# parrot-tts/Parrot-TTS

Hardware: AMD Instinct MI355X
Metric: audio samples/sec (16 kHz; see config.note) + RTF, 256-unit batch-64 per GPU (higher is better)
Workload: dtype f32 (f16x3 split products)

## Files before the change

parrot_tts_amd/csrc/conv_split.h:

```cpp
#pragma once
#include <cstdlib>
#include <type_traits>

#include "conv_mfma.h"

namespace parrot {

typedef short s16x8 __attribute__((ext_vector_type(8)));
typedef __bf16 bf16x8 __attribute__((ext_vector_type(8)));
typedef _Float16 f16x8 __attribute__((ext_vector_type(8)));

typedef __bf16 bf16x2 __attribute__((ext_vector_type(2)));
typedef _Float16 f16x2 __attribute__((ext_vector_type(2)));
typedef float f32x2 __attribute__((ext_vector_type(2)));
__device__ __forceinline__ unsigned pk_bf16(float x0, float x1) {
    const f32x2 v = {x0, x1};
    return __builtin_bit_cast(unsigned, __builtin_convertvector(v, bf16x2));
}
__device__ __forceinline__ unsigned pk_f16(float x0, float x1) {
    const f32x2 v = {x0, x1};
    return __builtin_bit_cast(unsigned, __builtin_convertvector(v, f16x2));
}
__device__ __forceinline__ float max_nc(float a, float b) {
    float r;
// ... 27 lines not shown
        const f32x2 v = {x0, x1};
        q[0] = __builtin_bit_cast(unsigned, __builtin_convertvector(v, f16x2));
        float r0, r1;
        asm("v_fma_mix_f32 %0, %1, -1.0, %2 op_sel_hi:[1,0,0]" : "=v"(r0) : "v"(q[0]), "v"(x0));
        asm("v_fma_mix_f32 %0, %1, -1.0, %2 op_sel:[1,0,0] op_sel_hi:[1,0,0]" : "=v"(r1) : "v"(q[0]), "v"(x1));
        q[1] = pk_f16(r0, r1);
    }
};
struct SchBf16 {
    static constexpr int ID = 3, NP = 1, NT = 1;
    static constexpr bool F16 = false;
    static constexpr float XS = 1.f;
    static constexpr int pa(int) { return 0; }
    static constexpr int pb(int) { return 0; }
    static constexpr int last_a(int) { return 0; }
    static __device__ __forceinline__ void split(float x0, float x1, unsigned (&q)[1]) { q[0] = pk_bf16(x0, x1); }
};
struct SchF16 {
    static constexpr int ID = 4, NP = 1, NT = 1;
    static constexpr bool F16 = true;
    static constexpr float XS = 8.f;
    static constexpr int pa(int) { return 0; }
    static constexpr int pb(int) { return 0; }
    static constexpr int last_a(int) { return 0; }
    static __device__ __forceinline__ void split(float x0, float x1, unsigned (&q)[1]) { q[0] = pk_f16(x0, x1); }
};

template <class SCH>
__device__ __forceinline__ f32x16 mfma32(const s16x8& a, const s16x8& b, const f32x16& c) {
    if constexpr (SCH::F16) return __builtin_amdgcn_mfma_f32_32x32x16_f16(__builtin_bit_cast(f16x8, a), __builtin_bit_cast(f16x8, b), c, 0, 0, 0);
    else return __builtin_amdgcn_mfma_f32_32x32x16_bf16(__builtin_bit_cast(bf16x8, a), __builtin_bit_cast(bf16x8, b), c, 0, 0, 0);
}
template <class SCH>
__device__ __forceinline__ f32x4 mfma16(const s16x8& a, const s16x8& b, const f32x4& c) {
    if constexpr (SCH::F16) return __builtin_amdgcn_mfma_f32_16x16x32_f16(__builtin_bit_cast(f16x8, a), __builtin_bit_cast(f16x8, b), c, 0, 0, 0);
    else return __builtin_amdgcn_mfma_f32_16x16x32_bf16(__builtin_bit_cast(bf16x8, a), __builtin_bit_cast(bf16x8, b), c, 0, 0, 0);
}
template <class SCH>
__device__ __forceinline__ float pre_scale(float v, float slope) {
    if constexpr (SCH::XS != 1.f) return max_nc(v * SCH::XS, v * (SCH::XS * slope));
    else return max_nc(v, v * slope);
}

template <int N, class F>
__device__ __forceinline__ void static_for(F&& f) {
    if constexpr (N > 0) {
        static_for<N - 1>(f);
        f(std::integral_constant<int, N - 1>{});
    }
}

template <class SCH, int WAVES_M, int WAVES_N, int WM, int WN, int MINW, int K, int SUBS = 1, bool LEAN = false>
__global__ __launch_bounds__(WAVES_M* WAVES_N * 64, MINW) void conv_split_kernel(const ConvParams p) {
    static_assert(SUBS == 1 || K == 1, "sub-slab staging: 1x1 convs only (no halo)");
    constexpr int NPC = SCH::NP, NTERM = SCH::NT;
    constexpr int NW = WAVES_M * WAVES_N, NT = NW * 64;
    constexpr int BM = WAVES_M * WM * 32;
    constexpr int BN = WAVES_N * WN * 32;
    constexpr int COLS = BN + ((SUBS > 1 && K == 1) ? 0 : CONV_HALO);
    constexpr int PIECE_BYTES = COLS * 32;
    constexpr int SUB_BYTES = NPC * PIECE_BYTES;
    constexpr int BUF_BYTES = SUBS * SUB_BYTES;
    constexpr int LIVE = SUBS * COLS * 2;
    constexpr int ITEMS = (LIVE + NT - 1) / NT;
    constexpr int KS = K * SUBS;
    constexpr int STEP_BYTES = NPC * 1024;

    extern __shared__ __attribute__((aligned(16))) char smem_raw[];

    const int tid = threadIdx.x;
    const int lane = tid & 63;
    const int wave = __builtin_amdgcn_readfirstlane(tid >> 6);
    const int wm = wave / WAVES_N;
    const int wn = wave % WAVES_N;
    const int half = lane >> 5;
    const int l31 = lane & 31;

    const int n_mb = (p.M + BM - 1) / BM;
    const int n_tiles = p.tiles_n * p.B, tpx = (n_tiles + 7) >> 3;
    const int xcd = blockIdx.x & 7, seq = blockIdx.x >> 3;
    const int mblock = seq % n_mb;
    const int tile_id = xcd * tpx + seq / n_mb;
    if (tile_id >= n_tiles || seq / n_mb >= tpx) return;
    const int b = tile_id / p.tiles_n;
    const int tn = tile_id - b * p.tiles_n;
    const int t0 = tn * BN;
    const int Tlim = p.row_len ? min(p.Tin, row_true_len(p.row_len[b], p.row_len_mul, p.row_len_add)) : p.Tin;
    const int W = BN + (p.k - 1) * p.dil;
    const int grp = (p.groups > 1) ? (mblock * BM) / p.Mg : 0;
    const float* __restrict__ xb = p.x + (size_t)b * p.x_bstride + (size_t)grp * p.Cin * p.Tin;

    static_assert(COLS % 64 == 0, "channel octet must be wave-uniform");
    const size_t xaddr = reinterpret_cast<size_t>(xb);
    const unsigned x_lo = __builtin_amdgcn_readfirstlane((unsigned)xaddr), x_hi = __builtin_amdgcn_readfirstlane((unsigned)(xaddr >> 32));
    const __amdgpu_buffer_rsrc_t xrsrc = __builtin_amdgcn_make_buffer_rsrc(
        reinterpret_cast<void*>(((size_t)x_hi << 32) | x_lo), 0, 0x7fffffff, 0x00020000);
    const int row_bytes = p.Tin * 4;
    const float slope = (p.pre == PRE_LRELU) ? p.pre_slope : 1.f;
    int voff[ITEMS], soct[ITEMS];
    static_for<ITEMS>([&](auto ic) {
        constexpr int i = decltype(ic)::value;
        const int item = tid + NT * i;
        const int so = item / COLS;
        const int col = item - so * COLS;
        const int tin = t0 - p.pad_left + col;
        voff[i] = (item < LIVE && col < W && tin >= 0 && tin < Tlim) ? tin * 4 : (int)0x80000000;
        soct[i] = __builtin_amdgcn_readfirstlane(min(so, 2 * SUBS - 1) * 8) * row_bytes;
// ... 23 lines not shown
                const int off = sub * SUB_BYTES + col * 32 + ((oct ^ ((col >> 3) & 1)) * 16);
#pragma unroll
                for (int pc = 0; pc < NPC; ++pc)
                    *reinterpret_cast<uint4*>(dst + pc * PIECE_BYTES + off) = uint4{q[0][pc], q[1][pc], q[2][pc], q[3][pc]};
            }
        });
    };

    f32x16 acc[WM][WN];
    const int m_wave = mblock * BM + wm * WM * 32;
    const int n_wave = t0 + wn * WN * 32;
    if constexpr (LEAN) conv_acc_init_lean<WM, WN>(p, acc, b, m_wave, n_wave, half, l31);
    else conv_acc_init<WM, WN>(p, acc, b, m_wave, n_wave, half, l31);

    const unsigned w_lo = __builtin_amdgcn_readfirstlane((unsigned)reinterpret_cast<size_t>(p.wfrag));
    const unsigned w_hi = __builtin_amdgcn_readfirstlane((unsigned)(reinterpret_cast<size_t>(p.wfrag) >> 32));
    const __amdgpu_buffer_rsrc_t wrsrc =
        __builtin_amdgcn_make_buffer_rsrc(reinterpret_cast<void*>(((size_t)w_hi << 32) | w_lo), 0, 0x7fffffff, 0x00020000);
    int abase[WM];
#pragma unroll
    for (int mt = 0; mt < WM; ++mt)
        abase[mt] = __builtin_amdgcn_readfirstlane((int)((mblock * (BM / 32) + wm * WM + mt) * p.n_it * STEP_BYTES));
    const unsigned lane16 = lane * 16;
    const int nsup = p.nchunks / SUBS;
    const int colbase = wn * WN * 32 + l31;
    auto load_b = [&](s16x8 (&bb)[WN][NPC], const char* __restrict__ xs, int tap) {
        const int col = colbase + tap * p.dil;
        const int off = col * 32 + ((half ^ ((col >> 3) & 1)) * 16);
#pragma unroll
        for (int nt = 0; nt < WN; ++nt)
#pragma unroll
            for (int pc = 0; pc < NPC; ++pc) bb[nt][pc] = *reinterpret_cast<const s16x8*>(xs + pc * PIECE_BYTES + nt * 1024 + off);
    };
    constexpr int TM = WM * WN, NMF = NTERM * TM;
    if constexpr (K > 0) {
        s16x8 A[2][WM][NPC], Bv[2][WN][NPC];
        auto load_a_piece = [&](s16x8 (&a)[WM][NPC], int pc, int soff) {
#pragma unroll
            for (int mt = 0; mt < WM; ++mt)
                a[mt][pc] = __builtin_bit_cast(s16x8, __builtin_amdgcn_raw_buffer_load_b128(wrsrc, lane16 + pc * 1024, abase[mt] + soff, 0));
        };
        auto next_chunk = [&](int q) { return (q + 1 == nsup) ? 0 : q + 1; };
        int cc = 0, cn = next_chunk(0);
#pragma unroll
        for (int pc = 0; pc < NPC; ++pc) {
            load_a_piece(A[0], pc, cc * KS * STEP_BYTES);
            load_a_piece(A[1], pc, (KS > 1 ? cc * KS + 1 : cn * KS) * STEP_BYTES);
        }
        load_slab(0);
        store_slab(0);
        __syncthreads();
        auto chunk = [&](auto par, int c) __attribute__((always_inline)) {
            constexpr int PAR = decltype(par)::value;
            const char* __restrict__ xs = smem_raw + (c & 1) * BUF_BYTES;
            const int cn2 = next_chunk(cn);
            load_slab(cn);
            load_b(Bv[PAR], xs, 0);
#pragma unroll
            for (int j = 0; j < KS; ++j) {
                const int cur = (PAR + j) & 1;
                const int tq = (j + 2 < KS) ? cc : (KS == 1 ? cn2 : cn);
                const int tj = (j + 2 < KS) ? j + 2 : (KS == 1 ? 0 : j + 2 - KS);
                const int soff = (tq * KS + tj) * STEP_BYTES;
                if (j + 1 < KS) load_b(Bv[cur ^ 1], xs + ((j + 1) / K) * SUB_BYTES, (j + 1) % K);
#pragma unroll
                for (int t = 0; t < NTERM; ++t) {
#pragma unroll
                    for (int mt = 0; mt < WM; ++mt)
#pragma unroll
                        for (int nt = 0; nt < WN; ++nt)
                            acc[mt][nt] = mfma32<SCH>(A[cur][mt][SCH::pa(t)], Bv[cur][nt][SCH::pb(t)], acc[mt][nt]);
#pragma unroll
                    for (int pc = 0; pc < NPC; ++pc)
                        if (t == SCH::last_a(pc)) load_a_piece(A[cur], pc, soff);
                }
            }
            constexpr int DS_START = (NPC >= 2) ? (SCH::last_a(NPC - 1) + 1) * TM - 1 + WM : 0;
            constexpr int SLAB_START = (NPC >= 2) ? (SCH::last_a(1) + 1) * TM - 1 + WM : 0;
            constexpr int SLAB_SLOTS = (NMF - SLAB_START) > 0 ? (NMF - SLAB_START) : 1, SLAB_PER = (ITEMS * 8 + SLAB_SLOTS - 1) / SLAB_SLOTS;
#pragma unroll
            for (int i = 0; i < NPC * WN; ++i) __builtin_amdgcn_sched_group_barrier(0x100, 1, 0);
#pragma unroll
            for (int j = 0; j < KS; ++j) {
                int ds_left = (j + 1 < KS) ? NPC * WN : 0, slab_left = (j == 0) ? ITEMS * 8 : 0;
#pragma unroll
                for (int m = 0; m < NMF; ++m) {
                    __builtin_amdgcn_sched_group_barrier(0x008, 1, 0);
#pragma unroll
                    for (int pc = NPC - 1; pc >= 1; --pc)
                        if (m >= (SCH::last_a(pc) + 1) * TM - 1 && m < (SCH::last_a(pc) + 1) * TM - 1 + WM) __builtin_amdgcn_sched_group_barrier(0x020, 1, 0);
                    if (m >= DS_START && ds_left > 0) {
                        __builtin_amdgcn_sched_group_barrier(0x100, 1, 0);
                        --ds_left;
                    }
                    if (m >= SLAB_START)
#pragma unroll
                        for (int q = 0; q < SLAB_PER; ++q)
                            if (slab_left > 0) {
                                __builtin_amdgcn_sched_group_barrier(0x020, 1, 0);
                                --slab_left;
                            }
                }
#pragma unroll
                for (int i = 0; i < WM; ++i) __builtin_amdgcn_sched_group_barrier(0x020, 1, 0);
            }
            __builtin_amdgcn_sched_barrier(0);
            store_slab((c + 1) & 1);
            __syncthreads();
            cc = cn;
            cn = cn2;
        };
        for (int c = 0; c < nsup; c += 2) {
            chunk(std::integral_constant<int, 0>{}, c);
            if (c + 1 < nsup) chunk(std::integral_constant<int, (KS & 1)>{}, c + 1);
        }
    } else {
        s16x8 a0[WM][NPC], b0[WN][NPC], a1[WM][NPC], b1[WN][NPC];
        auto load_a = [&](s16x8 (&a)[WM][NPC], int step) {
            const int soff = __builtin_amdgcn_readfirstlane(step) * STEP_BYTES;
#pragma unroll
            for (int mt = 0; mt < WM; ++mt)
#pragma unroll
                for (int pc = 0; pc < NPC; ++pc)
                    a[mt][pc] = __builtin_bit_cast(s16x8, __builtin_amdgcn_raw_buffer_load_b128(wrsrc, lane16 + pc * 1024, abase[mt] + soff, 0));
        };
        auto mfmas = [&](const s16x8 (&a)[WM][NPC], const s16x8 (&bb)[WN][NPC]) {
#pragma unroll
            for (int t = 0; t < NTERM; ++t)
#pragma unroll
                for (int mt = 0; mt < WM; ++mt)
#pragma unroll
                    for (int nt = 0; nt < WN; ++nt) acc[mt][nt] = mfma32<SCH>(a[mt][SCH::pa(t)], bb[nt][SCH::pb(t)], acc[mt][nt]);
        };
        load_a(a0, 0);
        load_slab(0);
        store_slab(0);
        __syncthreads();

        int cc = 0, cn = (1 == p.nchunks) ? 0 : 1;
        int c = 0, j = 0;
        const char* __restrict__ xs = smem_raw;
        auto step = [&](s16x8 (&xa)[WM][NPC], s16x8 (&xb)[WN][NPC], s16x8 (&ya)[WM][NPC], s16x8 (&yb)[WN][NPC]) {
            if (j == 0) {
                if (c + 1 < p.nchunks) load_slab(cn);
                load_b(xb, xs, 0);
            }
            const bool last_tap = (j + 1 == p.k);
            load_a(ya, last_tap ? cn * p.k : cc * p.k + j + 1);
            load_b(yb, xs, j + 1);
            mfmas(xa, xb);
            constexpr int MPER = (NMF / (NPC * (WM + WN))) > 0 ? (NMF / (NPC * (WM + WN))) : 1;
#pragma unroll
            for (int g = 0; g < WM * NPC; ++g) {
                __builtin_amdgcn_sched_group_barrier(0x008, MPER, 0);
                __builtin_amdgcn_sched_group_barrier(0x020, 1, 0);
            }
#pragma unroll
            for (int g = 0; g < WN * NPC; ++g) {
                __builtin_amdgcn_sched_group_barrier(0x008, MPER, 0);
                __builtin_amdgcn_sched_group_barrier(0x100, 1, 0);
            }
            __builtin_amdgcn_sched_barrier(0);
            if (last_tap) {
                if (c + 1 < p.nchunks) store_slab((c + 1) & 1);
                __syncthreads();
                ++c;
                xs = smem_raw + (c & 1) * BUF_BYTES;
                cc = cn;
                cn = (cc + 1 == p.nchunks) ? 0 : cc + 1;
                j = 0;
            } else {
                ++j;
            }
        };
        const int total = p.nchunks * p.k;
        for (int st = 0; st < total; st += 2) {
            step(a0, b0, a1, b1);
            if (st + 1 < total) step(a1, b1, a0, b0);
        }
    }
    if constexpr (LEAN) conv_epilogue_lean<WM, WN>(p, acc, b, m_wave, n_wave, half, l31);
    else conv_epilogue<WM, WN>(p, acc, b, m_wave, n_wave, half, l31);
}

template <class SCH, int WAVES_M, int WAVES_N, int WM, int WN, int MINW, int K, int SUBS = 1, bool LEAN = false>
inline hipError_t launch_conv_split_t(const ConvParams& p, dim3 grid, hipStream_t s) {
    constexpr int BN = WAVES_N * WN * 32;
    const size_t lds = (size_t)2 * SUBS * SCH::NP * (BN + ((SUBS > 1 && K == 1) ? 0 : CONV_HALO)) * 32;
    auto kern = conv_split_kernel<SCH, WAVES_M, WAVES_N, WM, WN, MINW, K, SUBS, LEAN>;
    static DynLdsOnce lds_once;
    {
        hipError_t e = ensure_dyn_lds(lds_once, reinterpret_cast<const void*>(kern), (size_t)lds);
        if (e != hipSuccess) return e;
    }
    hipLaunchKernelGGL(kern, grid, dim3(WAVES_M * WAVES_N * 64), lds, s, p);
    return hipGetLastError();
}

inline void split_tile(int variant, int& bm, int& bn) {
    if (variant == 2) { bm = 128; bn = 64; return; }
    if (variant == 3) { bm = 32; bn = 512; return; }
    bm = (variant & 1) ? 64 : 128;
    bn = (variant & 1) ? 256 : 128;
}
inline unsigned split_grid(const ConvParams& p, int bm) {
    const unsigned tiles = (unsigned)p.tiles_n * p.B, n_mb = (p.M + bm - 1) / bm;
    return (tiles + 7) / 8 * 8 * n_mb;
}
template <class SCH>
inline hipError_t launch_conv_split_s(int variant, const ConvParams& p, hipStream_t s) {
    int bm, bn;
    split_tile(variant, bm, bn);
    dim3 grid(split_grid(p, bm));
    if (variant == 3) return p.k == 3 ? launch_conv_split_t<SCH, 1, 4, 1, 4, 2, 3>(p, grid, s) : launch_conv_split_t<SCH, 1, 4, 1, 4, 2, 0>(p, grid, s);
    const bool lean = conv_lean_ok(p);
    if constexpr (SCH::ID == SchF16x3::ID) if (variant == 2) {
        if (p.k == 1 && p.nchunks % 4 == 0)
            return lean ? launch_conv_split_t<SCH, 4, 1, 1, 2, 3, 1, 4, true>(p, grid, s) : launch_conv_split_t<SCH, 4, 1, 1, 2, 3, 1, 4>(p, grid, s);
        switch (p.k) {
            case 1: return launch_conv_split_t<SCH, 4, 1, 1, 2, 3, 1>(p, grid, s);
            case 3: return launch_conv_split_t<SCH, 4, 1, 1, 2, 3, 3>(p, grid, s);
            case 9: return launch_conv_split_t<SCH, 4, 1, 1, 2, 3, 9>(p, grid, s);
            default: return launch_conv_split_t<SCH, 4, 1, 1, 2, 3, 0>(p, grid, s);
        }
    }
    if constexpr (SCH::ID != SchF16x3::ID) if (variant == 2) {
        if (p.k == 1 && p.nchunks % 4 == 0)
            return lean ? launch_conv_split_t<SCH, 2, 2, 2, 1, 3, 1, 4, true>(p, grid, s) : launch_conv_split_t<SCH, 2, 2, 2, 1, 3, 1, 4>(p, grid, s);
        switch (p.k) {
            case 1: return launch_conv_split_t<SCH, 2, 2, 2, 1, 3, 1>(p, grid, s);
            case 3: return launch_conv_split_t<SCH, 2, 2, 2, 1, 3, 3>(p, grid, s);
            case 9: return launch_conv_split_t<SCH, 2, 2, 2, 1, 3, 9>(p, grid, s);
            default: return launch_conv_split_t<SCH, 2, 2, 2, 1, 3, 0>(p, grid, s);
        }
    }
    if (variant & 1) switch (p.k) {
            case 1: return launch_conv_split_t<SCH, 1, 4, 2, 2, 2, 1>(p, grid, s);
            case 3: return launch_conv_split_t<SCH, 1, 4, 2, 2, 2, 3>(p, grid, s);
            case 7: return launch_conv_split_t<SCH, 1, 4, 2, 2, 2, 7>(p, grid, s);
            case 11: return launch_conv_split_t<SCH, 1, 4, 2, 2, 2, 11>(p, grid, s);
            default: return launch_conv_split_t<SCH, 1, 4, 2, 2, 2, 0>(p, grid, s);
        }
    switch (p.k) {
        case 3:
            return lean ? launch_conv_split_t<SCH, 2, 2, 2, 2, 2, 3, 1, true>(p, grid, s) : launch_conv_split_t<SCH, 2, 2, 2, 2, 2, 3>(p, grid, s);
        case 7: return launch_conv_split_t<SCH, 2, 2, 2, 2, 2, 7>(p, grid, s);
        case 9: return launch_conv_split_t<SCH, 2, 2, 2, 2, 2, 9>(p, grid, s);
        case 11: return launch_conv_split_t<SCH, 2, 2, 2, 2, 2, 11>(p, grid, s);
        default: return launch_conv_split_t<SCH, 2, 2, 2, 2, 2, 0>(p, grid, s);
    }
}
template <class SCH>
inline hipError_t launch_conv_split_generic(int variant, const ConvParams& p, hipStream_t s) {
    int bm, bn;
    split_tile(variant, bm, bn);
    dim3 grid(split_grid(p, bm));
    if (variant == 3) return launch_conv_split_t<SCH, 1, 4, 1, 4, 2, 0>(p, grid, s);
    if (variant == 2) {
        if (p.k == 1 && p.nchunks % 4 == 0) return launch_conv_split_t<SCH, 2, 2, 2, 1, 3, 1, 4>(p, grid, s);
        return launch_conv_split_t<SCH, 2, 2, 2, 1, 3, 0>(p, grid, s);
    }
    if (variant & 1) return launch_conv_split_t<SCH, 1, 4, 2, 2, 2, 0>(p, grid, s);
    return launch_conv_split_t<SCH, 2, 2, 2, 2, 2, 0>(p, grid, s);
}
hipError_t launch_conv_split_f16x3(int variant, const ConvParams& p, hipStream_t s);
hipError_t launch_conv_split_bf16x6(int variant, const ConvParams& p, hipStream_t s);
hipError_t launch_conv_split_bf16(int variant, const ConvParams& p, hipStream_t s);
hipError_t launch_conv_split_f16(int variant, const ConvParams& p, hipStream_t s);
inline hipError_t launch_conv_split(int scheme, int variant, const ConvParams& p, hipStream_t s) {
    switch (scheme) {
        case SchBf16x6::ID: return launch_conv_split_bf16x6(variant, p, s);
        case SchF16x3::ID: return launch_conv_split_f16x3(variant, p, s);
        case SchBf16::ID: return launch_conv_split_bf16(variant, p, s);
        case SchF16::ID: return launch_conv_split_f16(variant, p, s);
        default: return hipErrorInvalidValue;
    }
}

}
```

parrot_tts_amd/csrc/conv_valu.h:

```cpp
#pragma once
#include "conv_mfma.h"

namespace parrot {

struct ConvValuParams {
    const float* x;
    const float* w;
    const float* bias;
    float* y;
    int B, Cin, Tin, Tout;
    float slope;
    int act;
    const int32_t* row_len;
    int row_len_mul;
    int row_len_add;
    int* err;
};

__device__ __forceinline__ __amdgpu_buffer_rsrc_t valu_row_rsrc(const float* base) {
    const size_t a = reinterpret_cast<size_t>(base);
    const unsigned lo = __builtin_amdgcn_readfirstlane((unsigned)a), hi = __builtin_amdgcn_readfirstlane((unsigned)(a >> 32));
    return __builtin_amdgcn_make_buffer_rsrc(reinterpret_cast<void*>(((size_t)hi << 32) | lo), 0, 0x7fffffff, 0x00020000);
}

__global__ __launch_bounds__(256) void linear1_valu_kernel(const ConvValuParams p) {
    __shared__ float part[4][64];
    const int lane = threadIdx.x & 63, wave = threadIdx.x >> 6;
    const int b = blockIdx.y;
    const int t = blockIdx.x * 64 + lane;
    const int Tlim = p.row_len ? min(p.Tin, row_true_len(p.row_len[b], p.row_len_mul, p.row_len_add)) : p.Tin;
    const __amdgpu_buffer_rsrc_t xr = valu_row_rsrc(p.x + (size_t)b * p.Cin * p.Tin);
    const int voff = (t < Tlim) ? t * 4 : (int)0x80000000;
    const int per = (p.Cin + 3) / 4, c0 = wave * per, c1 = min(p.Cin, c0 + per);
    const int row_bytes = p.Tin * 4;
    float acc = 0.f;
    for (int c = c0; c < c1; ++c) {
        const float xv = __builtin_bit_cast(float, __builtin_amdgcn_raw_buffer_load_b32(xr, voff, c * row_bytes, 0));
        acc = fmaf(p.w[c], fmaxf(xv, xv * p.slope), acc);
    }
    part[wave][lane] = acc;
    __syncthreads();
    if (wave == 0 && t < p.Tout) {
        const float v = (((p.bias ? p.bias[0] : 0.f) + part[0][lane]) + part[1][lane]) + (part[2][lane] + part[3][lane]);
        if (p.act == ACT_TANH && p.err && !(fabsf(v) < INFINITY)) atomicExch(p.err, 5);
        p.y[(size_t)b * p.Tout + t] = (p.act == ACT_TANH) ? tanhf(v) : v;
    }
}

template <int K>
__global__ __launch_bounds__(256) void conv1_valu_kernel(const ConvValuParams p) {
    constexpr int NV = 4 + K - 1;
    const int b = blockIdx.y;
    const int t0 = (blockIdx.x * 256 + threadIdx.x) * 4;
    const int Tlim = p.row_len ? min(p.Tin, row_true_len(p.row_len[b], p.row_len_mul, p.row_len_add)) : p.Tin;
    const __amdgpu_buffer_rsrc_t xr = valu_row_rsrc(p.x + (size_t)b * p.Cin * p.Tin);
    int voff[NV];
#pragma unroll
    for (int i = 0; i < NV; ++i) {
        const int t = t0 - (K - 1) / 2 + i;
        voff[i] = (t >= 0 && t < Tlim) ? t * 4 : (int)0x80000000;
    }
    const float b0 = p.bias ? p.bias[0] : 0.f;
    float acc[4] = {b0, b0, b0, b0};
    const int row_bytes = p.Tin * 4;
    for (int c = 0; c < p.Cin; ++c) {
        float v[NV];
#pragma unroll
        for (int i = 0; i < NV; ++i) {
            const float xv = __builtin_bit_cast(float, __builtin_amdgcn_raw_buffer_load_b32(xr, voff[i], c * row_bytes, 0));
            v[i] = fmaxf(xv, xv * p.slope);
        }
#pragma unroll
        for (int j = 0; j < K; ++j) {
            const float wj = p.w[c * K + j];
#pragma unroll
            for (int o = 0; o < 4; ++o) acc[o] = fmaf(wj, v[o + j], acc[o]);
        }
    }
// ... 57 lines not shown
template <int COUT, int K, int U, int PAD>
__global__ __launch_bounds__(256) void convt_valu_kernel(const ConvValuParams p) {
    constexpr int DLO = -((K - 1 - PAD + U - 1) / U), DHI = (U - 1 + PAD) / U, ND = DHI - DLO + 1;
    const int b = blockIdx.y;
    const int n = blockIdx.x * 256 + threadIdx.x;
    const int Tlim = p.row_len ? min(p.Tin, row_true_len(p.row_len[b], p.row_len_mul, p.row_len_add)) : p.Tin;
    const __amdgpu_buffer_rsrc_t xr = valu_row_rsrc(p.x + (size_t)b * p.Cin * p.Tin);
    int voff[ND];
#pragma unroll
    for (int i = 0; i < ND; ++i) {
        const int t = n + DLO + i;
        voff[i] = (t >= 0 && t < Tlim) ? t * 4 : (int)0x80000000;
    }
    float acc[COUT][U];
#pragma unroll
    for (int o = 0; o < COUT; ++o)
#pragma unroll
        for (int ph = 0; ph < U; ++ph) acc[o][ph] = p.bias ? p.bias[o] : 0.f;
    const int row_bytes = p.Tin * 4;
    for (int c = 0; c < p.Cin; ++c) {
        float v[ND];
#pragma unroll
        for (int i = 0; i < ND; ++i) {
            const float xv = __builtin_bit_cast(float, __builtin_amdgcn_raw_buffer_load_b32(xr, voff[i], c * row_bytes, 0));
            v[i] = fmaxf(xv, xv * p.slope);
        }
        const float* __restrict__ wc = p.w + (size_t)c * COUT * K;
#pragma unroll
        for (int o = 0; o < COUT; ++o)
#pragma unroll
            for (int ph = 0; ph < U; ++ph)
#pragma unroll
                for (int kap = 0; kap < K; ++kap)
                    if ((ph + PAD - kap) % U == 0) acc[o][ph] = fmaf(wc[o * K + kap], v[(ph + PAD - kap) / U - DLO], acc[o][ph]);
    }
    if (n < p.Tin) {
        float* yb = p.y + (size_t)b * COUT * p.Tout;
        if (U == 2 && (p.Tout & 1) == 0 && n * 2 + 1 < p.Tout) {
            typedef float f32x2v __attribute__((ext_vector_type(2)));
#pragma unroll
            for (int o = 0; o < COUT; ++o) *reinterpret_cast<f32x2v*>(yb + (size_t)o * p.Tout + 2 * n) = f32x2v{acc[o][0], acc[o][U - 1]};
        } else {
#pragma unroll
            for (int o = 0; o < COUT; ++o)
#pragma unroll
                for (int ph = 0; ph < U; ++ph) {
                    const int t = n * U + ph;
                    if (t < p.Tout) yb[(size_t)o * p.Tout + t] = acc[o][ph];
                }
        }
    }
}

}
```

parrot_tts_amd/csrc/host_common.h:

```cpp
#pragma once
#include "../../include/parrot_hip_debug.h"

#include <hip/hip_runtime.h>

#include <memory>
#include <string>

#include "conv_consts.h"

namespace parrot {

int fail(int code, const std::string& msg);
}
#define HIP_TRY(expr)                                                                              \
    do {                                                                                           \
        hipError_t _e = (expr);                                                                    \
        if (_e != hipSuccess)                                                                      \
            return fail(PARROT_E_HIP, std::string(#expr) + ": " + hipGetErrorString(_e));          \
    } while (0)
#define TRY(expr)                \
    do {                         \
        int _r = (expr);         \
        if (_r != PARROT_OK) return _r; \
    } while (0)
// ... 46 lines not shown
    hipEvent_t a, b;
    int cfg;
    double flops, bytes;
};
bool prof_on();
int prof_open(ProfRec& rec, int row, double flops, double bytes, hipStream_t s);
int prof_close(ProfRec& rec, hipStream_t s);

int default_prec();
void query_device();
int num_cus();
struct CreateScope {
    int p0, f0, m0;
    CreateScope(int prec, int fused, int merge);
    ~CreateScope();
};
int create_prec();
int create_fused();
bool create_merge();
int resolve_parity_prec(int prec, const char* who, int* scheme);

struct DevFlag {
    int* p = nullptr;
    DevFlag() = default;
    DevFlag(const DevFlag&) = delete;
    ~DevFlag() { if (p) (void)hipFree(p); }
    int init();
    operator int*() const { return p; }
};
int check_flag(int* flag, hipStream_t s, int (*decode)(int status));
int model_status(const char* who, int status);
int status_async(int* flag, int32_t* dst_dev, hipStream_t s);
int peek_async(int* flag, int32_t* dst_dev, hipStream_t s, const char* who);

}

struct parrot_conv {
    parrot_conv_desc d{};
    int groups = 1;
    int M = 0, Mg = 0, Cout = 0, Cin = 0;
    int kk = 1, dil = 1, pad_left = 0, u = 1;
    int cfg = 0;
    int nchunks = 0, n_it = 0;
    float* wfrag = nullptr;
    float* bias = nullptr;
    int prec = 0;
    uint16_t* wfrag16 = nullptr;
    int n_it16 = 0;
    float wscale = 1.f;
    bool mfma16 = false;
    int* err_flag = nullptr;
    bool late_res = false;
    int valu_kind = 0;
    float* wraw = nullptr;

    ~parrot_conv() {
        if (wraw) (void)hipFree(wraw);
        if (wfrag16) (void)hipFree(wfrag16);
        if (wfrag) (void)hipFree(wfrag);
        if (bias) (void)hipFree(bias);
    }
    int out_len(int Tin) const {
        if (!d.transposed) return Tin + 2 * d.padding - d.dilation * (d.k - 1);
        return (Tin - 1) * d.stride - 2 * d.padding + d.k;
    }
};

namespace parrot {

struct PlaneArgs {
    const void* xplane = nullptr;
    void* yplane = nullptr;
    float yslope = 1.f;
    int plane_only = 0;
};
inline bool plane_ok(const parrot_conv* c) { return c && c->mfma16 && c->prec >= 1 && (c->kk == 7 || c->kk == 11) && c->M % 16 == 0 && c->Cin % 32 == 0; }
inline size_t plane_row_bytes(int prec, int C, int T) { return (size_t)(prec == PARROT_PREC_F16X3 ? 2 : 1) * 2 * C * T; }
struct RowLens {
    const int32_t* len = nullptr;
    int mul = 1, add = 0;
};
struct ConvOpts {
    RowLens rows;
    PlaneArgs planes;
};

int conv_build(parrot_conv** out, const parrot_conv_desc* d, int groups, const float* w, const float* bias, bool allow16 = true);
int make_conv(std::unique_ptr<parrot_conv>& slot, int cin, int cout, int k, int dil, int pad, int transposed, int stride, int pre, float slope,
              int act, const float* w, const float* b, int groups = 1, bool allow16 = true);
int upload(float** dst, const float* src, size_t n);
int conv_launch(const parrot_conv* c, const float* x, const float* res, float* y, int B, int Tin, int epi, float div, hipStream_t s,
                const ConvOpts& o = ConvOpts());

}
```

parrot_tts_amd/csrc/host_conv.hip:

```cpp
#include "host_common.h"

#include <algorithm>
#include <cstdio>
#include <cstring>
#include <vector>

#include "conv_split.h"
#include "conv_split16.h"
#include "conv_mfma16.h"
#include "conv_valu.h"
#include "kernels_conv.h"
#include "weight_pack.h"

using namespace parrot;
static_assert(SchBf16x6::ID == PARROT_PREC_BF16X6 && SchF16x3::ID == PARROT_PREC_F16X3 && SchBf16::ID == PARROT_PREC_BF16 && SchF16::ID == PARROT_PREC_F16,
              "weight_pack.h reads a scheme off its PARROT_PREC_* number");

static int choose_cfg(int M, int k) {
    if (M <= 16) return 6;
    if (M <= 32) return 2;
    if (M <= 64) return 1;
    return (k <= 3) ? 3 : 0;
}

static bool valu_kernels_enabled() {
    static const bool on = [] { const char* e = getenv("PARROT_VALU_KERNELS"); return !e || atoi(e) != 0; }();
    return on;
}
static bool mfma16_enabled() {
    static const bool on = [] { const char* e = getenv("PARROT_MFMA16"); return !e || atoi(e) != 0; }();
    return on;
}
static int small_tiles_mode() {
    static const int m = [] { const char* e = getenv("PARROT_SMALL_TILES"); return e ? atoi(e) : 2; }();
    return m;
}

int parrot::conv_build(parrot_conv** out, const parrot_conv_desc* d, int groups, const float* w, const float* bias, bool allow16) {
    if (!out || !d || !w) return fail(PARROT_E_INVALID, "conv_create: null argument");
    if (d->c_in <= 0 || d->c_out <= 0 || d->k <= 0 || d->dilation <= 0 || groups <= 0 || d->c_in % groups || d->c_out % groups)
        return fail(PARROT_E_INVALID, "conv_create: bad dimensions");
    std::unique_ptr<parrot_conv> c(new parrot_conv());
    c->d = *d;
    c->groups = groups;
    c->Cout = d->c_out;
    c->Cin = d->c_in / groups;
    int dmin = 0;
    if (d->transposed) {
        if (d->stride > 64) return fail(PARROT_E_UNSUPPORTED, "conv_create: transposed stride > 64");
        if (groups != 1 || d->dilation != 1 || d->stride <= 0) return fail(PARROT_E_UNSUPPORTED, "conv_create: transposed conv needs groups=1, dilation=1");
        const int u = d->stride, p = d->padding, k = d->k;
        int dlo = 1 << 30, dhi = -(1 << 30);
        for (int r = 0; r < u; ++r)
            for (int kap = 0; kap < k; ++kap)
                if ((r + p - kap) % u == 0) {
                    int dl = (r + p - kap) / u;
                    dlo = std::min(dlo, dl);
                    dhi = std::max(dhi, dl);
                }
        if (dlo > dhi) return fail(PARROT_E_INVALID, "conv_create: transposed conv has no taps");
        dmin = dlo;
        c->u = u;
        c->kk = dhi - dlo + 1;
        c->dil = 1;
        c->pad_left = -dlo;
        c->M = d->c_out * u;
    } else {
        if (d->stride > 1) return fail(PARROT_E_UNSUPPORTED, "conv_create: strided Conv1d is not on the path");
        c->u = 1;
        c->kk = d->k;
        c->dil = d->dilation;
        c->pad_left = d->padding;
        c->M = d->c_out;
    }
    c->Mg = c->M / groups;
    if ((c->kk - 1) * c->dil > CONV_HALO) return fail(PARROT_E_UNSUPPORTED, "conv_create: (k-1)*dilation exceeds the LDS halo (64)");
    c->cfg = (d->tile_cfg >= 0) ? d->tile_cfg : choose_cfg(c->Mg, c->kk);
    if (c->cfg >= NUM_TILE_CFGS) return fail(PARROT_E_INVALID, "conv_create: tile_cfg out of range");
    if (c->cfg == 6 && (d->transposed || groups != 1 || c->M > 16)) {
        if (d->tile_cfg == 6) return fail(PARROT_E_UNSUPPORTED, "conv_create: the 16-row tile needs a plain conv with <= 16 output channels");
        c->cfg = 2;
    }
    const TileCfg t = tile_cfg(c->cfg);
    if (groups > 1 && c->Mg % t.bm) return fail(PARROT_E_UNSUPPORTED, "conv_create: rows per group must be a multiple of the tile height");
    const int CI = t.ci, QN = CI / 8;
    c->nchunks = (c->Cin + CI - 1) / CI;
    c->n_it = c->cfg == 6 ? c->nchunks * c->kk : c->nchunks * c->kk * QN;
    const int kk = c->kk;
    const GemmWeights W{w, c->M, c->Cin, d->k, d->transposed != 0, d->c_out, c->u, d->padding, dmin};
    const int want_prec = (d->precision >= 0) ? d->precision : create_prec();
    if (want_prec > PARROT_PREC_F16) return fail(PARROT_E_INVALID, "conv_create: unknown precision");
    const bool slope_ok = d->pre_act != PRE_LRELU || (d->pre_slope >= 0.f && d->pre_slope <= 1.f);
    if (want_prec >= 1 && c->Mg >= 32 && d->tile_cfg < 0 && c->Cin % 16 == 0 && slope_ok) {
        c->prec = want_prec;
        c->cfg = (c->Mg <= 32) ? 2 : (c->Mg <= 64) ? 1 : 0;
        const TileCfg t16 = tile_cfg(c->cfg);
        if (groups > 1 && c->Mg % t16.bm) return fail(PARROT_E_UNSUPPORTED, "conv_create: rows per group must be a multiple of the tile height");
        if (scheme_is_f16(want_prec)) c->wscale = f16_weight_scale(w, (size_t)d->c_in / groups * d->c_out * d->k);
        c->mfma16 = allow16 && mfma16_enabled() && split16_has(want_prec, c->kk) && !d->transposed && groups == 1 && c->Cin % 32 == 0 && c->M >= 64;
        int rows = 32, bm = t16.bm;
        if (c->mfma16) {
            int bn16;
            rows = 16;
            split16_tile(c->M >= 128 ? 0 : 1, bm, bn16);
        }
        const int chans = 512 / rows;
        c->nchunks = (c->Cin + chans - 1) / chans;
        c->n_it16 = c->nchunks * c->kk;
        const size_t n_steps = (size_t)((c->M + bm - 1) / bm * (bm / rows)) * c->n_it16;
        const size_t n16 = (n_steps + 1) * scheme_pieces(want_prec) * 512;
        if (n16 * sizeof(uint16_t) >= ((size_t)1 << 31)) return fail(PARROT_E_UNSUPPORTED, "conv_create: packed weight stream larger than 2 GiB");
        std::vector<uint16_t> pk16(n16, 0);
        const int n_it16 = c->n_it16;
        pack_pieces(pk16.data(), n_steps, want_prec, c->wscale, W, [=](size_t st, int lane, int e) {
            const int mt = (int)(st / n_it16), ch = (int)(st % n_it16) / kk, j = (int)(st % n_it16) % kk;
            return WeightAt{mt * rows + lane % rows, ch * chans + 8 * (lane / rows) + e, j};
        });
        HIP_TRY(hipMalloc((void**)&c->wfrag16, pk16.size() * sizeof(uint16_t)));
        HIP_TRY(hipMemcpy(c->wfrag16, pk16.data(), pk16.size() * sizeof(uint16_t), hipMemcpyHostToDevice));
    } else {
        const size_t n_steps = c->cfg == 6 ? (size_t)c->n_it : (size_t)((c->M + t.bm - 1) / t.bm * (t.bm / 32)) * c->n_it;
        std::vector<float> pk((n_steps + 1) * 256, 0.f);
        if (c->cfg == 6)
            pack_f32(pk.data(), n_steps, W, [=](size_t st, int lane, int e) { return WeightAt{lane & 15, (int)st / kk * 16 + 4 * e + (lane >> 4), (int)st % kk}; });
        else {
            const int n_it = c->n_it;
            pack_f32(pk.data(), n_steps, W, [=](size_t st, int lane, int e) {
                const int mt = (int)(st / n_it), r = (int)(st % n_it), q = r % QN, j = r / QN % kk, ch = r / QN / kk;
                return WeightAt{mt * 32 + (lane & 31), ch * CI + 8 * q + 2 * e + (lane >> 5), j};
            });
        }
        HIP_TRY(hipMalloc((void**)&c->wfrag, pk.size() * sizeof(float)));
        HIP_TRY(hipMemcpy(c->wfrag, pk.data(), pk.size() * sizeof(float), hipMemcpyHostToDevice));
    }
    if (d->tile_cfg < 0 && groups == 1 && slope_ok && d->dilation == 1 && valu_kernels_enabled()) {
        if (!d->transposed && d->c_out == 1 && ((d->k == 7 && d->padding == 3) || (d->k == 1 && d->padding == 0)) &&
            (d->act == ACT_NONE || d->act == ACT_TANH))
            c->valu_kind = 1;
        if (d->transposed && d->c_out == 16 && d->k == 4 && d->stride == 2 && d->padding == 1 && d->act == ACT_NONE) c->valu_kind = 2;
        if (c->valu_kind) {
            const size_t n = (size_t)d->c_in * d->c_out * d->k;
            HIP_TRY(hipMalloc((void**)&c->wraw, n * sizeof(float)));
            HIP_TRY(hipMemcpy(c->wraw, w, n * sizeof(float), hipMemcpyHostToDevice));
        }
    }
    if (bias) {
        HIP_TRY(hipMalloc((void**)&c->bias, (size_t)d->c_out * sizeof(float)));
        HIP_TRY(hipMemcpy(c->bias, bias, (size_t)d->c_out * sizeof(float), hipMemcpyHostToDevice));
    }
    *out = c.release();
    return PARROT_OK;
}

int parrot::conv_launch(const parrot_conv* c, const float* x, const float* res, float* y, int B, int Tin, int epi, float div, hipStream_t s,
                        const ConvOpts& o) {
    const PlaneArgs& pl = o.planes;
    if (B <= 0 || Tin <= 0) return fail(PARROT_E_INVALID, "conv_run: empty batch or sequence");
    const int Tout = c->out_len(Tin);
    if (Tout <= 0) return fail(PARROT_E_INVALID, "conv_run: sequence shorter than the kernel");
    if (c->valu_kind && !res && epi == EPI_STORE && (double)c->d.c_in * Tin * 4.0 < 2147483648.0) {
        ConvValuParams q{};
        q.x = x; q.w = c->wraw; q.bias = c->bias; q.y = y;
        q.B = B; q.Cin = c->d.c_in; q.Tin = Tin; q.Tout = Tout;
        q.slope = c->d.pre_act == PRE_LRELU ? c->d.pre_slope : 1.f;
        q.act = c->d.act;
        q.row_len = o.rows.len; q.row_len_mul = o.rows.mul; q.row_len_add = o.rows.add;
        q.err = c->err_flag;
        ProfRec rec{};
        const double macs = (double)B * c->d.c_out * c->d.c_in * c->d.k * (c->d.transposed ? (double)Tin : (double)Tout);
        if (prof_on()) TRY(prof_open(rec, c->valu_kind == 1 ? PROF_VALU_CONV1 : PROF_VALU_CONVT, 2.0 * macs, 4.0 * B * ((double)c->d.c_in * Tin + (double)c->d.c_out * Tout), s));
        if (c->valu_kind == 1 && c->d.k == 7 && (Tin & 3) == 0 && (reinterpret_cast<size_t>(x) & 15) == 0 && (reinterpret_cast<size_t>(y) & 15) == 0)
            hipLaunchKernelGGL(conv1_valu7_vec_kernel, dim3((Tout + 1023) / 1024, B), dim3(256), 0, s, q);
        else if (c->valu_kind == 1 && c->d.k == 7) hipLaunchKernelGGL(conv1_valu_kernel<7>, dim3((Tout + 1023) / 1024, B), dim3(256), 0, s, q);
        else if (c->valu_kind == 1) hipLaunchKernelGGL(linear1_valu_kernel, dim3((Tout + 63) / 64, B), dim3(256), 0, s, q);
        else hipLaunchKernelGGL((convt_valu_kernel<16, 4, 2, 1>), dim3((Tin + 255) / 256, B), dim3(256), 0, s, q);
        HIP_TRY(hipGetLastError());
        if (prof_on()) TRY(prof_close(rec, s));
        return PARROT_OK;
    }
    ConvParams p{};
    p.x = x; p.wfrag = c->wfrag; p.bias = c->bias; p.res = res; p.y = y;
    p.B = B; p.Cin = c->Cin; p.Tin = Tin; p.M = c->M; p.Cout = c->Cout;
    p.Ncols = (c->u > 1) ? (Tout + c->u - 1) / c->u : Tout;
    p.Tout = Tout;
    p.k = c->kk; p.dil = c->dil; p.pad_left = c->pad_left;
    p.nchunks = c->nchunks; p.n_it = c->n_it;
    p.pre = c->d.pre_act; p.pre_slope = c->d.pre_slope; p.act = c->d.act;
    p.epi = epi; p.div = div; p.u = c->u; p.u_inv16 = (65536 + c->u - 1) / c->u;
    p.groups = c->groups; p.Mg = c->Mg;
    p.row_len = o.rows.len; p.row_len_mul = o.rows.mul; p.row_len_add = o.rows.add;
    p.acc_scale = p.out_scale = 1.f;
    p.lean = 1;
    p.n_cus = num_cus();
    p.fold_res = c->late_res ? 0 : 1;
    if (pl.xplane || pl.yplane) {
        if (!plane_ok(c) || (pl.yplane && epi != EPI_STORE)) return fail(PARROT_E_INVALID, "conv_run: operand planes need a conv_split16 layer (k = 7 / 11) and EPI_STORE");
        p.xplane = pl.xplane; p.yplane = pl.yplane;
        p.xplane_bstride = (long)plane_row_bytes(c->prec, c->Cin, Tin);
        p.yplane_bstride = (long)plane_row_bytes(c->prec, c->M, Tout);
        p.yplane_slope = pl.yslope; p.plane_only = pl.plane_only;
    }
    p.x_bstride = (long)c->d.c_in * Tin;
    p.y_bstride = (long)c->Cout * Tout;
    p.res_bstride = p.y_bstride;
    int cfg = c->cfg;
    if (c->prec == 0 && (cfg == 0 || cfg == 3) && p.Ncols <= 64 && tile_cfg(4).ci == tile_cfg(cfg).ci) cfg = 4;
    if (c->prec >= 1) {
        p.wfrag = reinterpret_cast<const float*>(c->wfrag16);
        p.n_it = c->n_it16;
        p.acc_scale = scheme_xs(c->prec) * c->wscale;
        p.out_scale = 1.f / p.acc_scale;
        if ((double)c->Cin * Tin * 4.0 >= 2147483648.0) return fail(PARROT_E_UNSUPPORTED, "conv_run: batch row larger than 2 GiB");
    }
    TileCfg t = tile_cfg(cfg);
    int variant16 = 0;
    const bool small_tiles = small_tiles_mode() >= 1;
    if (c->mfma16) {
        variant16 = c->M >= 128 ? 0 : 1;
        split16_tile(variant16, t.bm, t.bn, c->kk);
        if (small_tiles && (long)((p.Ncols + t.bn - 1) / t.bn) * B * ((c->M + t.bm - 1) / t.bm) < num_cus()) {
            variant16 += 2;
            split16_tile(variant16, t.bm, t.bn, c->kk);
            if (small_tiles_mode() >= 2 && (long)((p.Ncols + t.bn - 1) / t.bn) * B * ((c->M + t.bm - 1) / t.bm) * 2 <= num_cus() && c->M >= 128) variant16 = 3;
        } else if (small_tiles && p.Ncols <= 64) variant16 += 2;
        else if (variant16 == 0 && split16_wide_fits(p.Ncols, B, (c->M + 127) / 128, num_cus())) variant16 = 4;
        split16_tile(variant16, t.bm, t.bn, c->kk);
        if ((double)c->M * Tout * 4.0 >= 2147483648.0) return fail(PARROT_E_UNSUPPORTED, "conv_run: output row tile larger than 2 GiB");
        {
            auto al16 = [](const void* q, long stride) { return (reinterpret_cast<size_t>(q) & 15) == 0 && (stride & 3) == 0; };
            p.epi16 = (Tout % 4 == 0) && al16(y, p.y_bstride) && (!res || al16(res, p.res_bstride));
        }
    } else if (c->prec >= 1) {
        const bool few = small_tiles && cfg == 0 && (c->kk == 3 || c->kk == 9) && (long)((p.Ncols + 127) / 128) * B * ((c->M + 127) / 128) < num_cus();
        variant16 = (cfg == 2) ? 3 : (cfg == 0 && (c->kk == 1 || p.Ncols <= 64 || few)) ? 2 : cfg;
        split_tile(variant16, t.bm, t.bn);
    }
    p.tiles_n = (p.Ncols + t.bn - 1) / t.bn;
    ProfRec rec{};
    if (prof_on()) {
        const double macs = (double)B * c->d.c_out * c->Cin * c->d.k * (c->d.transposed ? (double)Tin : (double)Tout);
        const double elems = (double)B * ((double)c->d.c_in * Tin + (double)c->Cout * Tout * (1 + (res ? 1 : 0) + (epi != EPI_STORE ? 1 : 0)));
        const int row = c->mfma16 ? (variant16 == 4 ? PROF_SPLIT16_WIDE : (variant16 & 1) ? PROF_SPLIT16_ODD : PROF_SPLIT16)
                                  : (c->prec >= 1) ? (variant16 == 2 ? PROF_SPLIT_V2 : variant16 == 3 ? PROF_SPLIT_V3 : PROF_SPLIT + cfg) : cfg;
        TRY(prof_open(rec, row, 2.0 * macs, 4.0 * (elems + (double)c->d.c_out * c->Cin * c->d.k), s));
    }
    HIP_TRY(c->mfma16 ? launch_conv_split16(c->prec, variant16, p, s) : c->prec >= 1 ? launch_conv_split(c->prec, variant16, p, s) : (cfg == 6 ? launch_conv_mfma16(p, s) : launch_conv(cfg, p, s)));
    if (c->d.act == ACT_TANH) {
        const size_t n = (size_t)B * c->Cout * Tout;
        hipLaunchKernelGGL(tanh_inplace_kernel, dim3((unsigned)((n + 255) / 256)), dim3(256), 0, s, y, n, c->err_flag);
        HIP_TRY(hipGetLastError());
    }
    if (prof_on()) TRY(prof_close(rec, s));
    return PARROT_OK;
}

int parrot::upload(float** dst, const float* src, size_t n) {
    HIP_TRY(hipMalloc((void**)dst, n * sizeof(float)));
    HIP_TRY(hipMemcpy(*dst, src, n * sizeof(float), hipMemcpyHostToDevice));
    return PARROT_OK;
}

int parrot::make_conv(std::unique_ptr<parrot_conv>& slot, int cin, int cout, int k, int dil, int pad, int transposed, int stride, int pre,
                      float slope, int act, const float* w, const float* b, int groups, bool allow16) {
    parrot_conv_desc d{};
    d.c_in = cin; d.c_out = cout; d.k = k; d.dilation = dil; d.padding = pad; d.transposed = transposed; d.stride = stride;
    d.pre_act = pre; d.pre_slope = slope; d.act = act; d.tile_cfg = -1; d.precision = -1;
    parrot_conv* c = nullptr;
    TRY(conv_build(&c, &d, groups, w, b, allow16));
    slot.reset(c);
    return PARROT_OK;
}

extern "C" int parrot_conv_create(parrot_conv_t** out, const parrot_conv_desc* d, const float* w_host, const float* bias_host) {
    return conv_build(out, d, 1, w_host, bias_host);
}
extern "C" void parrot_conv_destroy(parrot_conv_t* c) { delete c; }
extern "C" int parrot_conv_out_len(const parrot_conv_t* c, int32_t T_in) { return c ? c->out_len(T_in) : PARROT_E_INVALID; }
extern "C" int parrot_conv_num_tile_cfgs(void) { return NUM_TILE_CFGS; }
extern "C" int parrot_conv_run(parrot_conv_t* c, const float* x, const float* res, float* y, int32_t B, int32_t T_in,
                               int32_t epilogue, float div, void* stream) {
    if (!c || !x || !y) return fail(PARROT_E_INVALID, "conv_run: null argument");
    if (epilogue < 0 || epilogue > 2) return fail(PARROT_E_INVALID, "conv_run: bad epilogue");
    if (epilogue == EPI_STORE && y != x && y != res && c->out_len(T_in) > 0)
        TRY(poison(y, (size_t)B * c->Cout * c->out_len(T_in) * sizeof(float), (hipStream_t)stream));
    return conv_launch(c, x, res, y, B, T_in, epilogue, div, (hipStream_t)stream);
}

extern "C" int parrot_selftest(void* stream) {
    float* d = nullptr;
    HIP_TRY(hipMalloc((void**)&d, 64 * 16 * sizeof(float)));
    hipLaunchKernelGGL(mfma_probe_kernel, dim3(1), dim3(64), 0, (hipStream_t)stream, d);
    std::vector<float> h(64 * 16);
    hipError_t e = hipMemcpy(h.data(), d, h.size() * sizeof(float), hipMemcpyDeviceToHost);
    (void)hipFree(d);
    if (e != hipSuccess) return fail(PARROT_E_HIP, hipGetErrorString(e));
    for (int lane = 0; lane < 64; ++lane)
        for (int r = 0; r < 16; ++r) {
            const int row = (r & 3) + 8 * (r >> 2) + 4 * (lane >> 5), col = lane & 31;
            const float want = (float)(col + 1) * (float)(1001 * row + 100000);
// ... 9 lines not shown
```

Baseline: 301.6 million.

## Add sub-slab single-buffer split kernel for k=3 upsample convs and packed convT VALU kernel

Adds a conv_split variant that stages four input sub-slabs for k=3 transposed convs through a single LDS buffer, taking more channels per stage with fewer chunk iterations. The single buffer needs an extra barrier before each store, and the slab prefetch is no longer interleaved with the MFMAs. It also adds a transposed-conv VALU kernel for the 16-output k=4 stride-2 layer. That kernel uses host-permuted weights, packed f32x2 FMAs and double-buffered input fetches. Both paths are on by default and can be turned off with the PARROT_UPSAMPLE environment variable.

Result: no change. 302.9 million (median of 6 runs) (+0.4%).

```diff
diff --git a/parrot_tts_amd/csrc/conv_split.h b/parrot_tts_amd/csrc/conv_split.h
--- a/parrot_tts_amd/csrc/conv_split.h
+++ b/parrot_tts_amd/csrc/conv_split.h
@@ -103,7 +103,8 @@
 
 template <class SCH, int WAVES_M, int WAVES_N, int WM, int WN, int MINW, int K, int SUBS = 1, bool LEAN = false>
 __global__ __launch_bounds__(WAVES_M* WAVES_N * 64, MINW) void conv_split_kernel(const ConvParams p) {
-    static_assert(SUBS == 1 || K == 1, "sub-slab staging: 1x1 convs only (no halo)");
+    static_assert(SUBS == 1 || K > 0, "sub-slab staging: straight-line kernels only");
+    constexpr bool ONEBUF = SUBS > 1 && K > 1;
     constexpr int NPC = SCH::NP, NTERM = SCH::NT;
     constexpr int NW = WAVES_M * WAVES_N, NT = NW * 64;
     constexpr int BM = WAVES_M * WM * 32;
@@ -233,9 +234,10 @@
         __syncthreads();
         auto chunk = [&](auto par, int c) __attribute__((always_inline)) {
             constexpr int PAR = decltype(par)::value;
-            const char* __restrict__ xs = smem_raw + (c & 1) * BUF_BYTES;
+            const char* __restrict__ xs = smem_raw + (ONEBUF ? 0 : (c & 1) * BUF_BYTES);
             const int cn2 = next_chunk(cn);
-            load_slab(cn);
+            const bool more = c + 1 < nsup;
+            if (!ONEBUF || more) load_slab(cn);
             load_b(Bv[PAR], xs, 0);
 #pragma unroll
             for (int j = 0; j < KS; ++j) {
@@ -263,7 +265,7 @@
             for (int i = 0; i < NPC * WN; ++i) __builtin_amdgcn_sched_group_barrier(0x100, 1, 0);
 #pragma unroll
             for (int j = 0; j < KS; ++j) {
-                int ds_left = (j + 1 < KS) ? NPC * WN : 0, slab_left = (j == 0) ? ITEMS * 8 : 0;
+                int ds_left = (j + 1 < KS) ? NPC * WN : 0, slab_left = (j == 0 && !ONEBUF) ? ITEMS * 8 : 0;
 #pragma unroll
                 for (int m = 0; m < NMF; ++m) {
                     __builtin_amdgcn_sched_group_barrier(0x008, 1, 0);
@@ -286,8 +288,16 @@
                 for (int i = 0; i < WM; ++i) __builtin_amdgcn_sched_group_barrier(0x020, 1, 0);
             }
             __builtin_amdgcn_sched_barrier(0);
-            store_slab((c + 1) & 1);
-            __syncthreads();
+            if constexpr (ONEBUF) {
+                if (more) {
+                    __syncthreads();
+                    store_slab(0);
+                    __syncthreads();
+                }
+            } else {
+                store_slab((c + 1) & 1);
+                __syncthreads();
+            }
             cc = cn;
             cn = cn2;
         };
@@ -367,7 +377,7 @@
 template <class SCH, int WAVES_M, int WAVES_N, int WM, int WN, int MINW, int K, int SUBS = 1, bool LEAN = false>
 inline hipError_t launch_conv_split_t(const ConvParams& p, dim3 grid, hipStream_t s) {
     constexpr int BN = WAVES_N * WN * 32;
-    const size_t lds = (size_t)2 * SUBS * SCH::NP * (BN + ((SUBS > 1 && K == 1) ? 0 : CONV_HALO)) * 32;
+    const size_t lds = (size_t)((SUBS > 1 && K > 1) ? 1 : 2) * SUBS * SCH::NP * (BN + ((SUBS > 1 && K == 1) ? 0 : CONV_HALO)) * 32;
     auto kern = conv_split_kernel<SCH, WAVES_M, WAVES_N, WM, WN, MINW, K, SUBS, LEAN>;
     static DynLdsOnce lds_once;
     {
@@ -448,7 +458,9 @@
 hipError_t launch_conv_split_bf16x6(int variant, const ConvParams& p, hipStream_t s);
 hipError_t launch_conv_split_bf16(int variant, const ConvParams& p, hipStream_t s);
 hipError_t launch_conv_split_f16(int variant, const ConvParams& p, hipStream_t s);
+hipError_t launch_conv_split_sub4(int variant, const ConvParams& p, hipStream_t s);
 inline hipError_t launch_conv_split(int scheme, int variant, const ConvParams& p, hipStream_t s) {
+    if (variant >= 4) return (variant == 4 && scheme == SchF16x3::ID && p.k == 3 && p.nchunks % 4 == 0) ? launch_conv_split_sub4(variant, p, s) : hipErrorInvalidValue;
     switch (scheme) {
         case SchBf16x6::ID: return launch_conv_split_bf16x6(variant, p, s);
         case SchF16x3::ID: return launch_conv_split_f16x3(variant, p, s);
diff --git a/parrot_tts_amd/csrc/conv_valu.h b/parrot_tts_amd/csrc/conv_valu.h
--- a/parrot_tts_amd/csrc/conv_valu.h
+++ b/parrot_tts_amd/csrc/conv_valu.h
@@ -23,7 +23,7 @@
     return __builtin_amdgcn_make_buffer_rsrc(reinterpret_cast<void*>(((size_t)hi << 32) | lo), 0, 0x7fffffff, 0x00020000);
 }
 
-__global__ __launch_bounds__(256) void linear1_valu_kernel(const ConvValuParams p) {
+static __global__ __launch_bounds__(256) void linear1_valu_kernel(const ConvValuParams p) {
     __shared__ float part[4][64];
     const int lane = threadIdx.x & 63, wave = threadIdx.x >> 6;
     const int b = blockIdx.y;
@@ -187,4 +187,68 @@
     }
 }
 
-}
+constexpr int CONVT_PK_COUT = 16, CONVT_PK_AHEAD = 4;
+inline void convt_pk_pack(float* dst, const float* w, int Cin) {
+    static const int perm[4] = {1, 0, 3, 2};
+    for (int i = 0; i < Cin * CONVT_PK_COUT; ++i)
+        for (int e = 0; e < 4; ++e) dst[4 * i + e] = w[4 * i + perm[e]];
+}
+template <int G>
+__global__ __launch_bounds__(256) void convt_valu_pk_kernel(const ConvValuParams p) {
+    typedef float f32x2v __attribute__((ext_vector_type(2)));
+    constexpr int COUT = CONVT_PK_COUT;
+    const int b = blockIdx.y;
+    const int n = blockIdx.x * 256 + threadIdx.x;
+    const int Tlim = p.row_len ? min(p.Tin, row_true_len(p.row_len[b], p.row_len_mul, p.row_len_add)) : p.Tin;
+    const __amdgpu_buffer_rsrc_t xr = valu_row_rsrc(p.x + (size_t)b * p.Cin * p.Tin);
+    int voff[3];
+#pragma unroll
+    for (int i = 0; i < 3; ++i) {
+        const int t = n - 1 + i;
+        voff[i] = (t >= 0 && t < Tlim) ? t * 4 : (int)0x80000000;
+    }
+    f32x2v acc[COUT];
+#pragma unroll
+    for (int o = 0; o < COUT; ++o) acc[o] = f32x2v{0.f, 0.f};
+    if (p.bias) {
+#pragma unroll
+        for (int o = 0; o < COUT; ++o) acc[o] = f32x2v{p.bias[o], p.bias[o]};
+    }
+    const int row_bytes = p.Tin * 4;
+    float xa[G][3], xb[G][3];
+    auto fetch = [&](float (&xs)[G][3], int c0) __attribute__((always_inline)) {
+#pragma unroll
+        for (int g = 0; g < G; ++g)
+#pragma unroll
+            for (int i = 0; i < 3; ++i) xs[g][i] = __builtin_bit_cast(float, __builtin_amdgcn_raw_buffer_load_b32(xr, voff[i], (c0 + g) * row_bytes, 0));
+    };
+    auto fmas = [&](const float (&xs)[G][3], int c0) __attribute__((always_inline)) {
+#pragma unroll
+        for (int g = 0; g < G; ++g) {
+            float v[3];
+#pragma unroll
+            for (int i = 0; i < 3; ++i) v[i] = fmaxf(xs[g][i], xs[g][i] * p.slope);
+            const f32x2v* __restrict__ wc = reinterpret_cast<const f32x2v*>(p.w) + (size_t)(c0 + g) * COUT * 2;
+#pragma unroll
+            for (int o = 0; o < COUT; ++o) {
+                acc[o] = __builtin_elementwise_fma(wc[2 * o], f32x2v{v[1], v[2]}, acc[o]);
+                acc[o] = __builtin_elementwise_fma(wc[2 * o + 1], f32x2v{v[0], v[1]}, acc[o]);
+            }
+        }
+    };
+    fetch(xa, 0);
+    for (int c0 = 0; c0 < p.Cin; c0 += 2 * G) {
+        fetch(xb, c0 + G);
+        fmas(xa, c0);
+        fetch(xa, min(c0 + 2 * G, p.Cin - G));
+        fmas(xb, c0 + G);
+    }
+    if (n < p.Tin) {
+        float* yb = p.y + (size_t)b * COUT * p.Tout + 2 * (size_t)n;
+#pragma unroll
+        for (int o = 0; o < COUT; ++o) *reinterpret_cast<f32x2v*>(yb + (size_t)o * p.Tout) = acc[o];
+    }
+}
+hipError_t launch_convt_valu_pk(const ConvValuParams& p, hipStream_t s);
+
+}
diff --git a/parrot_tts_amd/csrc/host_common.h b/parrot_tts_amd/csrc/host_common.h
--- a/parrot_tts_amd/csrc/host_common.h
+++ b/parrot_tts_amd/csrc/host_common.h
@@ -122,7 +122,9 @@
     int* err_flag = nullptr;
     bool late_res = false;
     int valu_kind = 0;
+    bool convt_pk = false;
     float* wraw = nullptr;
+    bool sub4 = false;
 
     ~parrot_conv() {
         if (wraw) (void)hipFree(wraw);
diff --git a/parrot_tts_amd/csrc/host_conv.hip b/parrot_tts_amd/csrc/host_conv.hip
--- a/parrot_tts_amd/csrc/host_conv.hip
+++ b/parrot_tts_amd/csrc/host_conv.hip
@@ -34,6 +34,10 @@
 static int small_tiles_mode() {
     static const int m = [] { const char* e = getenv("PARROT_SMALL_TILES"); return e ? atoi(e) : 2; }();
     return m;
+}
+static bool upsample_kernels_enabled() {
+    const char* e = getenv("PARROT_UPSAMPLE");
+    return !e || atoi(e) != 0;
 }
 
 int parrot::conv_build(parrot_conv** out, const parrot_conv_desc* d, int groups, const float* w, const float* bias, bool allow16) {
@@ -104,6 +108,7 @@
             rows = 16;
             split16_tile(c->M >= 128 ? 0 : 1, bm, bn16);
         }
+        c->sub4 = upsample_kernels_enabled() && d->transposed && want_prec == PARROT_PREC_F16X3 && c->kk == 3 && c->Cin % 64 == 0 && c->Cin <= 128 && c->cfg == 0;
         const int chans = 512 / rows;
         c->nchunks = (c->Cin + chans - 1) / chans;
         c->n_it16 = c->nchunks * c->kk;
@@ -140,8 +145,11 @@
         if (d->transposed && d->c_out == 16 && d->k == 4 && d->stride == 2 && d->padding == 1 && d->act == ACT_NONE) c->valu_kind = 2;
         if (c->valu_kind) {
             const size_t n = (size_t)d->c_in * d->c_out * d->k;
+            c->convt_pk = c->valu_kind == 2 && d->c_in % (2 * CONVT_PK_AHEAD) == 0 && upsample_kernels_enabled();
+            std::vector<float> pk(c->convt_pk ? n : 0);
+            if (c->convt_pk) convt_pk_pack(pk.data(), w, d->c_in);
             HIP_TRY(hipMalloc((void**)&c->wraw, n * sizeof(float)));
-            HIP_TRY(hipMemcpy(c->wraw, w, n * sizeof(float), hipMemcpyHostToDevice));
+            HIP_TRY(hipMemcpy(c->wraw, c->convt_pk ? pk.data() : w, n * sizeof(float), hipMemcpyHostToDevice));
         }
     }
     if (bias) {
@@ -173,6 +181,7 @@
             hipLaunchKernelGGL(conv1_valu7_vec_kernel, dim3((Tout + 1023) / 1024, B), dim3(256), 0, s, q);
         else if (c->valu_kind == 1 && c->d.k == 7) hipLaunchKernelGGL(conv1_valu_kernel<7>, dim3((Tout + 1023) / 1024, B), dim3(256), 0, s, q);
         else if (c->valu_kind == 1) hipLaunchKernelGGL(linear1_valu_kernel, dim3((Tout + 63) / 64, B), dim3(256), 0, s, q);
+        else if (c->convt_pk) HIP_TRY(launch_convt_valu_pk(q, s));
         else hipLaunchKernelGGL((convt_valu_kernel<16, 4, 2, 1>), dim3((Tin + 255) / 256, B), dim3(256), 0, s, q);
         HIP_TRY(hipGetLastError());
         if (prof_on()) TRY(prof_close(rec, s));
@@ -235,6 +244,7 @@
         variant16 = (cfg == 2) ? 3 : (cfg == 0 && (c->kk == 1 || p.Ncols <= 64 || few)) ? 2 : cfg;
         split_tile(variant16, t.bm, t.bn);
     }
+    const int variant_run = (!c->mfma16 && c->sub4 && variant16 == 0) ? 4 : variant16;
     p.tiles_n = (p.Ncols + t.bn - 1) / t.bn;
     ProfRec rec{};
     if (prof_on()) {
@@ -244,7 +254,7 @@
                                   : (c->prec >= 1) ? (variant16 == 2 ? PROF_SPLIT_V2 : variant16 == 3 ? PROF_SPLIT_V3 : PROF_SPLIT + cfg) : cfg;
         TRY(prof_open(rec, row, 2.0 * macs, 4.0 * (elems + (double)c->d.c_out * c->Cin * c->d.k), s));
     }
-    HIP_TRY(c->mfma16 ? launch_conv_split16(c->prec, variant16, p, s) : c->prec >= 1 ? launch_conv_split(c->prec, variant16, p, s) : (cfg == 6 ? launch_conv_mfma16(p, s) : launch_conv(cfg, p, s)));
+    HIP_TRY(c->mfma16 ? launch_conv_split16(c->prec, variant16, p, s) : c->prec >= 1 ? launch_conv_split(c->prec, variant_run, p, s) : (cfg == 6 ? launch_conv_mfma16(p, s) : launch_conv(cfg, p, s)));
     if (c->d.act == ACT_TANH) {
         const size_t n = (size_t)B * c->Cout * Tout;
         hipLaunchKernelGGL(tanh_inplace_kernel, dim3((unsigned)((n + 255) / 256)), dim3(256), 0, s, y, n, c->err_flag);
diff --git a/parrot_tts_amd/csrc/tu_upsample.hip b/parrot_tts_amd/csrc/tu_upsample.hip
--- /dev/null
+++ b/parrot_tts_amd/csrc/tu_upsample.hip
@@ -0,0 +1,13 @@
+#include "conv_split.h"
+#include "conv_valu.h"
+namespace parrot {
+hipError_t launch_conv_split_sub4(int variant, const ConvParams& p, hipStream_t s) {
+    int bm, bn;
+    split_tile(variant, bm, bn);
+    return launch_conv_split_t<SchF16x3, 2, 2, 2, 2, 2, 3, 4>(p, dim3(split_grid(p, bm)), s);
+}
+hipError_t launch_convt_valu_pk(const ConvValuParams& p, hipStream_t s) {
+    hipLaunchKernelGGL((convt_valu_pk_kernel<CONVT_PK_AHEAD>), dim3((p.Tin + 255) / 256, p.B), dim3(256), 0, s, p);
+    return hipGetLastError();
+}
+}
```
